# ibejarano/Pynama

Measured on AMD Instinct MI355X. Metric: assembled element-DOFs/sec + CG iterations/sec, 10M-DOF Poisson, 1/2/4/8 MI355X, higher is better.
Workload: dtype f64

## Files before the change

### include/pynama_hip.h

```cpp
#ifndef PYNAMA_HIP_H
#define PYNAMA_HIP_H

#include <stdint.h>

#ifdef __cplusplus
extern "C" {
#endif

typedef struct pyn_ctx pyn_ctx;

enum {
  PYN_OK = 0,
  PYN_EINVAL = -1,
  PYN_EHIP = -2,
  PYN_ENCCL = -3,
  PYN_ENOTCONV = -4,
  PYN_ENOGPU = -5
};

enum { PYN_Q_FULL = 0, PYN_Q_RED = 1, PYN_Q_NODAL = 2 };

enum {
  PYN_FORM_LAPLACE = 0,
  PYN_FORM_MASS_NODAL = 1,
// ... 92 lines not shown
};
#define PYN_FIELD_MAX_PARAMS 4
int pyn_field_info(int field, int* dim, int* bs, int* nparams);
int pyn_field_eval(pyn_ctx* ctx, int field, const double* params, int nparams, int set_id, int vec_id);
int pyn_vec_set_nodes(pyn_ctx* ctx, int vec_id, int set_id, const double* values, int nvalues, const uint8_t* dofs);

int pyn_assemble_kle(pyn_ctx* ctx, double alpha_d, double alpha_w, int K, int Krhs, int Rw, int Rd,
                     int variant);
int pyn_assemble_kle_noslip(pyn_ctx* ctx, double alpha_d, double alpha_w, const int* mat_ids);
int pyn_assemble_scalar(pyn_ctx* ctx, int form, int A, int Arhs, int variant);
int pyn_elem_local(pyn_ctx* ctx, int form, double alpha_d, double alpha_w, const double* corners,
                   double* out0, double* out1, double* out2);

int pyn_assemble_operator(pyn_ctx* ctx, int rule, int nterms, const int32_t* terms, const double* coef, int mat_id);
int pyn_elem_operator_local(pyn_ctx* ctx, int rule, int br, int bc, int nterms, const int32_t* terms,
                            const double* coef, const double* corners, double* out);

int pyn_spmv(pyn_ctx* ctx, int mat_id, int x_vec, int y_vec);
int pyn_product_last(pyn_ctx* ctx, int64_t* info);
int pyn_product_choose(int br, int bc, int npat, int maxw, int64_t nnzb, int64_t n_owned, int rhs_compact, int solver, int image,
                       int sell_image, int block_sell, int no_csrlb, int no_sell, double bcsr_min_avg, int bcsr_lanes, int bcsr_unroll,
                       int* kind, int* W, int* lanes, int* unroll);
int pyn_assemble_last(pyn_ctx* ctx, int64_t* info);
int pyn_assemble_choose(const int64_t* request, const int64_t* facts, const int64_t* knobs, int64_t* out);
int pyn_assemble_choose_layout(char* buf, int len);
enum { PYN_MATFREE_OFF = 0, PYN_MATFREE_LAPLACE = 1, PYN_MATFREE_KLE = 2, PYN_MATFREE_KLE_GENERAL = 3,
       PYN_MATFREE_KLE_NGL3_GENERAL = 4 };
int pyn_matfree_set(pyn_ctx* ctx, int op, double alpha_d, double alpha_w);
int pyn_matfree_apply(pyn_ctx* ctx, int op, int x_vec, int y_vec);
typedef struct pyn_solve_opts {
  int method;
  int pc;
  int norm_type;
  int maxit;
  int restart;
  int fixed_iters;
  int profile;
  int cg_variant;
  int gmres_orthog;
  int matfree;
  double rtol, atol, dtol;
} pyn_solve_opts;
typedef struct pyn_solve_info {
  int iters;
  int reason;
  double rnorm;
// ... 50 lines not shown
```

### pynama_amd/_lib.py

```python
from __future__ import annotations

import ctypes as C
import os
import subprocess
import sys

import numpy as np

_HERE = os.path.dirname(os.path.abspath(__file__))
LIB_PATH = os.environ.get("PYNAMA_LIB_PATH") or os.path.join(_HERE, "libpynama_hip.so")
CSRC = os.path.join(_HERE, "csrc")

Q_FULL, Q_RED, Q_NODAL = 0, 1, 2
FORM_LAPLACE, FORM_MASS_NODAL, FORM_MASS_FULL, FORM_KLE, FORM_OPERATOR = 0, 1, 2, 3, 4
KSP_CG, KSP_GMRES = 0, 1
MATFREE_OFF, MATFREE_LAPLACE, MATFREE_KLE, MATFREE_KLE_GENERAL, MATFREE_KLE_NGL3_GENERAL = 0, 1, 2, 3, 4
PC_NONE, PC_JACOBI, PC_MG = 0, 1, 2
MG_MAX_LEVELS = 16
TS_MAX_STAGES = 8
NORM_PRECONDITIONED, NORM_UNPRECONDITIONED, NORM_NATURAL = 0, 1, 2
T_SYMBOLIC, T_ASSEMBLE, T_SPMV, T_SOLVE = 0, 1, 2, 3
(FIELD_TG2D_VEL, FIELD_TG2D_VORT, FIELD_TG3D_VEL, FIELD_TG3D_VORT, FIELD_TG3D_CONV, FIELD_TG3D_DIFF,
 FIELD_SEN2D_VEL, FIELD_SEN2D_VORT, FIELD_SEN2D_CONV, FIELD_SEN2D_DIFF) = range(10)
FIELD_COUNT, FIELD_MAX_PARAMS = 10, 4


class PynamaHipError(RuntimeError):
    pass


class SolveOpts(C.Structure):
    _fields_ = [("method", C.c_int), ("pc", C.c_int), ("norm_type", C.c_int), ("maxit", C.c_int),
                ("restart", C.c_int), ("fixed_iters", C.c_int), ("profile", C.c_int), ("cg_variant", C.c_int),
# ... 68 lines not shown
    "pyn_vec_axpby": [_P, _I, _D, _I, _D, _I],
    "pyn_vec_pointwise_mult": [_P, _I, _I, _I],
    "pyn_vec_reciprocal": [_P, _I],
    "pyn_vec_vtensv": [_P, _I, _I],
    "pyn_vec_dot": [_P, _I, _I, C.POINTER(_D)],
    "pyn_vec_norm": [_P, _I, _I, C.POINTER(_D)],
    "pyn_vec_maxpy": [_P, _I, _I, _I, _pi32, _pf64],
    "pyn_ts_step_finish": [_P, _I, _I, _pi32, _pf64, _P, _D, _D, C.POINTER(_D)],
    "pyn_nodeset_create": [_P, _L, _P, C.POINTER(_I)],
    "pyn_nodeset_destroy": [_P, _I],
    "pyn_field_info": [_I, C.POINTER(_I), C.POINTER(_I), C.POINTER(_I)],
    "pyn_field_eval": [_P, _I, _pf64, _I, _I, _I],
    "pyn_vec_set_nodes": [_P, _I, _I, _pf64, _I, _P],
    "pyn_assemble_kle": [_P, _D, _D, _I, _I, _I, _I, _I],
    "pyn_assemble_kle_noslip": [_P, _D, _D, C.POINTER(_I)],
    "pyn_assemble_scalar": [_P, _I, _I, _I, _I],
    "pyn_elem_local": [_P, _I, _D, _D, _pf64, _P, _P, _P],
    "pyn_assemble_operator": [_P, _I, _I, _pi32, _pf64, _I],
    "pyn_elem_operator_local": [_P, _I, _I, _I, _I, _pi32, _pf64, _pf64, _pf64],
    "pyn_spmv": [_P, _I, _I, _I],
    "pyn_product_last": [_P, _pi64],
    "pyn_product_choose": [_I] * 4 + [_L, _L] + [_I] * 7 + [_D, _I, _I] + [C.POINTER(_I)] * 4,
    "pyn_assemble_last": [_P, _pi64],
    "pyn_assemble_choose": [_pi64, _pi64, _pi64, _pi64],
    "pyn_assemble_choose_layout": [C.c_char_p, _I],
    "pyn_matfree_apply": [_P, _I, _I, _I],
    "pyn_matfree_set": [_P, _I, _D, _D],
    "pyn_solve": [_P, _I, _I, _I, C.POINTER(SolveOpts), C.POINTER(SolveInfo)],
    "pyn_direct_max_rows": [],
    "pyn_solve_direct": [_P, _I, _I, _I, C.POINTER(SolveInfo)],
    "pyn_direct_band_info": [_P, _I, C.POINTER(_L), C.POINTER(_L), C.POINTER(_L)],
    "pyn_solve_direct_band": [_P, _I, _I, _I, _L, C.POINTER(SolveInfo)],
    "pyn_mg_setup": [_P, _I, C.POINTER(MgOpts)],
    "pyn_mg_info": [_P, _I, C.POINTER(_I), _pi64, _pf64, C.POINTER(_D), C.POINTER(_I)],
    "pyn_mg_apply": [_P, _I, _I, _I],
    "pyn_mg_level_get": [_P, _I, _I, _pf64],
    "pyn_ibm_set": [_P, _I, _I, _L, _pf64, _pf64, _pf64, _pf64],
    "pyn_ibm_interp": [_P, _I, _pf64],
    "pyn_ibm_spread": [_P, _pf64, _I],
    "pyn_ibm_correct": [_P, _I, _pf64, _pf64],
    "pyn_ibm_matrix_get": [_P, _pf64],
    "pyn_ibm_info": [_P, _pi64],
    "pyn_ibm_clear": [_P],
    "pyn_probe_create": [_P, _L, _pf64, C.POINTER(_I)],
    "pyn_probe_info": [_P, _I, _pi64],
    "pyn_probe_get": [_P, _I, _pi32, _pf64],
# ... 2 lines not shown
    "pyn_timers_get": [_P, _pf64, _I],
}

_lib = None


def build_library(force=False):
    if force:
        subprocess.check_call(["make", "-C", CSRC, "clean"])
    subprocess.check_call(["make", "-C", CSRC, "-j4"])
    return LIB_PATH


def load_library():
    global _lib
    if _lib is not None:
        return _lib
    if not os.path.exists(LIB_PATH):
        raise PynamaHipError(
            f"{LIB_PATH} not found: build it with `python -c 'import __graft_entry__ as g; g.build()'` "
            "(or `make -C pynama_amd/csrc`). pynama_amd has no CPU fallback.")
    lib = C.CDLL(LIB_PATH)
    for name, args in SIGNATURES.items():
        fn = getattr(lib, name)
        fn.argtypes = args
        fn.restype = C.c_int
    for name in ("pyn_last_error", "pyn_source_hash"):
        getattr(lib, name).argtypes = []
        getattr(lib, name).restype = C.c_char_p
    _lib = lib
    return lib


def _check(rc):
    if rc != 0:
        raise PynamaHipError(f"[{rc}] {_lib.pyn_last_error().decode(errors='replace')}")


def source_hash() -> str:
    return load_library().pyn_source_hash().decode()


def alloc_live():
    n, b = _L(0), _L(0)
    _check(load_library().pyn_alloc_live(C.byref(n), C.byref(b)))
    return n.value, b.value
# ... 425 lines not shown
        _check(self.lib.pyn_elem_local(self.h, form, 0.0, 0.0, c, o0.ctypes.data_as(_P), None, None))
        return o0

    def assemble_operator(self, rule, terms, coef, mid):
        t = _i32(terms).reshape(-1, 3)
        _check(self.lib.pyn_assemble_operator(self.h, rule, t.shape[0], t, _f64(coef), mid))

    def elem_operator_local(self, rule, br, bc, terms, coef, corners):
        t = _i32(terms).reshape(-1, 3)
        out = np.empty((br * self.nn, bc * self.nn))
        _check(self.lib.pyn_elem_operator_local(self.h, rule, br, bc, t.shape[0], t, _f64(coef), _f64(corners).ravel(), out))
        return out

    def spmv(self, mid, x, y):
        _check(self.lib.pyn_spmv(self.h, mid, x, y))

    def product_last(self):
        info = np.zeros(8, np.int64)
        _check(self.lib.pyn_product_last(self.h, info))
        keys = ("family", "param", "unroll", "dot", "grid", "npat", "maxw", "launches")
        return {k: int(v) for k, v in zip(keys, info)}

    def assemble_last(self):
        info = np.zeros(8, np.int64)
        _check(self.lib.pyn_assemble_last(self.h, info))
        return {k: int(v) for k, v in zip(_ASM_LAST_KEYS, info)}

    def mesh_ho_lattice(self):
        g, a, b, c = _I(0), _I(0), _I(0), _I(0)
        _check(self.lib.pyn_mesh_ho_lattice(self.h, C.byref(g), C.byref(a), C.byref(b), C.byref(c)))
        return g.value, a.value, b.value, c.value

    def matfree_apply(self, x, y, op=1):
        _check(self.lib.pyn_matfree_apply(self.h, op, x, y))

    def matfree_set(self, op=1, alpha_d=0.0, alpha_w=0.0):
        _check(self.lib.pyn_matfree_set(self.h, op, alpha_d, alpha_w))

    def matfree_kle_set(self, alpha_d, alpha_w):
        self.matfree_set(MATFREE_KLE, alpha_d, alpha_w)

    def solve(self, mid, b, x, method=KSP_CG, pc=PC_JACOBI, rtol=1e-5, atol=1e-50, dtol=1e5, maxit=10000,
              restart=30, norm_type=NORM_PRECONDITIONED, fixed_iters=0, profile=0, cg_variant=0, gmres_orthog=0,
              matfree=0) -> SolveInfo:
        o = SolveOpts(method, pc, norm_type, maxit, restart, fixed_iters, profile, cg_variant, gmres_orthog, matfree,
                      rtol, atol, dtol)
        info = SolveInfo()
        _check(self.lib.pyn_solve(self.h, mid, b, x, C.byref(o), C.byref(info)))
        return info
# ... 132 lines not shown
```

### pynama_amd/csrc/pyn_assemble.hip

```cpp
#include <cstring>

#include "pyn_internal.h"

namespace {

struct AsmArgs {
  const int32_t* conn;
  const double* xyz;
  int64_t n_elem, n_owned;
  int dim, nn, nc;
  int ngp[3];
  const double* w[3];
  const double* H[3];
  const double* Hrs[3];
  const double* HrsCoo[3];
  const int32_t* rowptr;
  const int32_t* colidx;
  const uint8_t* bcmask;
  int form;
  double alpha_d, alpha_w;
  double *K, *Krhs, *Rw, *Rd;
  double *Kfs, *Krhsfs, *Rwfs, *Rdfs;
  const int32_t *rcrow, *rcrow_fs;
  const int32_t* esel;
// ... 950 lines not shown
}

int zero_blocks(pyn_ctx* c, double* val, int64_t blocks, int br, int bc) {
  if (val) PYN_HIP(hipMemsetAsync(val, 0, (size_t)blocks * br * bc * sizeof(double), c->stream));
  return PYN_OK;
}

void launch_bc_identity(pyn_ctx* c, int ndof, double* K, double* Krhs, double* Kfs, double* Krhsfs, const int32_t* rcrow,
                        const int32_t* rcrow_fs) {
  const int64_t n = c->n_owned * ndof;
  const int grid = (int)std::min<int64_t>((n + 255) / 256, 4096);
  bc_identity_kernel<<<grid, 256, 0, c->stream>>>(c->d_rowptr, c->d_colidx, c->d_bcmask, c->n_owned, ndof, K, Krhs, Kfs, Krhsfs, rcrow, rcrow_fs);
}

int asm_finish(pyn_ctx* c, const AsmPlan& P, const AsmRequest& rq) {
  PYN_HIP(hipEventRecord(c->ev1, c->stream));
  PYN_HIP(hipStreamSynchronize(c->stream));
  float ms = 0;
  PYN_HIP(hipEventElapsedTime(&ms, c->ev0, c->ev1));
  c->timers[PYN_T_ASSEMBLE] = ms;
  const int64_t r[7] = {P.kind, P.shape, P.k_closed, P.rw_closed, P.kind == AK_GENERIC ? rq.generic : 0, rq.krhs_completed, rq.dinv_written};
  std::copy(r, r + 7, c->asm_last);
  c->asm_last[7] += 1;
  return PYN_OK;
}

bool rowrun_asked(const AsmRequest& rq) {
  if (rq.variant == 0 || rq.Rd) return false;
  return rq.form == PYN_FORM_KLE ? rq.K || (rq.Rw && !rq.Krhs) : rq.form == PYN_FORM_LAPLACE && rq.K && !rq.Rw;
}
bool rowrun_static(const AsmRequest& rq, const AsmFacts& f, const AsmKnobs& k) {
  if (!f.ho3_valid || f.ho3_tabs_nn != f.nn || f.ngp0 < 1) return false;
  if (rq.form == PYN_FORM_OPERATOR)
    return rq.op_rule == PYN_Q_NODAL && f.ho3_tabs_ok2 && rq.op_nterms <= PYN_HO3_MAX_TERMS && !k.no_ho3_operator;
  return rowrun_asked(rq) && f.ho3_tabs_ok0 && !(f.ngl == 2 && f.dim == 3) && (rq.form != PYN_FORM_KLE || f.ho3_tabs_ok1);
}
bool lattice_static(const AsmRequest& rq, const AsmFacts& f) {
  return rq.variant != 0 && rq.form == PYN_FORM_LAPLACE && rq.K && !rq.Rw && !rq.Rd && f.lat_valid && !f.plan0_user && f.ngp0 == 8;
}
bool kle_lattice_static(const AsmRequest& rq, const AsmFacts& f, const AsmKnobs& k) {
  return rq.variant != 0 && rq.form == PYN_FORM_KLE && (rq.K || (rq.Rw && !rq.Krhs)) && !rq.Rd && !f.plan1_user && f.lat_valid &&
         f.ngp0 == 8 && f.ngp1 == 1 && !k.no_kle_lattice;
}
bool patch_static(const AsmRequest& rq, const AsmFacts& f, const AsmKnobs& k) {
  if (rq.variant == 0 || !rq.K || rq.Rd || f.dim != 3) return false;
  if (rq.form == PYN_FORM_KLE) return f.nn == 8 && f.ngp0 == 8 && f.ngp1 == 1;
// ... 272 lines not shown
  rq.variant = variant;
  rq.rhs_clean = Arhs != Aid && rhs_is_clean(c, k, Arhs);
  PYN_TRY(mat_ptr(c, Aid, 1, 1, "A", &rq.K));
  PYN_TRY(mat_ptr(c, Arhs, 1, 1, "Arhs", &rq.Krhs, &rq.rcrow));
  if (rq.rcrow) rq.rhs_clean = false;
  rq.krhs_blocks = rhs_blocks(c, Arhs);
  if (Aid >= 0 && form == PYN_FORM_LAPLACE && !k.no_dinv) {
    DMat& m = c->mats[Aid];
    if (!m.dinv) PYN_HIP(m.dinv.alloc((size_t)c->n_owned));
    rq.dinv = m.dinv;
  }
  PYN_TRY(asm_run(c, rq, k));
  if (rq.dinv_written) c->mats[Aid].dinv_valid = true;
  if (rq.Krhs && rq.K) c->mats[Arhs].rhs_clean = c->bc_stamp;
  return PYN_OK;
}

extern "C" int pyn_assemble_last(pyn_ctx* c, int64_t* info) {
  PYN_CHECK(c && info, "NULL argument");
  std::copy(c->asm_last, c->asm_last + 8, info);
  return PYN_OK;
}

#define PYN_ASM_REQUEST "form,variant,K,Krhs,Rw,Rd,krhs_compact,op_rule,op_nterms"
extern "C" int pyn_assemble_choose_layout(char* buf, int len) {
#define PYN_X(f) #f ","
#define PYN_F(f, e) #f ","
#define PYN_I(f, e, d) #f ","
  const char* layout = "request:" PYN_ASM_REQUEST ";facts:" PYN_ASM_FACTS(PYN_X) ";knobs:" PYN_ASM_KNOBS(PYN_F, PYN_I);
#undef PYN_X
#undef PYN_F
#undef PYN_I
  PYN_CHECK(buf && len > (int)strlen(layout), "pyn_assemble_choose_layout: the buffer needs %zu bytes", strlen(layout) + 1);
  strcpy(buf, layout);
  return PYN_OK;
}

extern "C" int pyn_assemble_choose(const int64_t* request, const int64_t* facts, const int64_t* knobs, int64_t* out) {
  PYN_CHECK(request && facts && knobs && out, "pyn_assemble_choose: NULL argument");
  static double target;
  static const int32_t crow = 0;
  AsmRequest rq;
  rq.form = (int)request[0];
  rq.variant = (int)request[1];
  rq.K = request[2] ? &target : nullptr;
  rq.Krhs = request[3] ? &target : nullptr;
// ... 121 lines not shown
```

### pynama_amd/csrc/pyn_assemble_lattice.hip

```cpp
#include "pyn_internal.h"
#include "pyn_q1_hex.h"
#include "pyn_lattice.h"

namespace {


__device__ __forceinline__ double lat_affine_inv(const double* __restrict__ S, const double (&E)[3][3], double (&Ji)[3][3]) {
  double J[3][3];
#pragma unroll
  for (int d = 0; d < 3; ++d)
#pragma unroll
    for (int x = 0; x < 3; ++x) J[d][x] = fma(S[d * 3 + 2], E[2][x], fma(S[d * 3 + 1], E[1][x], S[d * 3] * E[0][x]));
  const double c00 = J[1][1] * J[2][2] - J[1][2] * J[2][1];
  const double c01 = J[1][2] * J[2][0] - J[1][0] * J[2][2];
  const double c02 = J[1][0] * J[2][1] - J[1][1] * J[2][0];
  const double det = J[0][0] * c00 + J[0][1] * c01 + J[0][2] * c02;
  const double r = 1.0 / det;
  Ji[0][0] = c00 * r;
  Ji[0][1] = (J[0][2] * J[2][1] - J[0][1] * J[2][2]) * r;
  Ji[0][2] = (J[0][1] * J[1][2] - J[0][2] * J[1][1]) * r;
  Ji[1][0] = c01 * r;
  Ji[1][1] = (J[0][0] * J[2][2] - J[0][2] * J[2][0]) * r;
  Ji[1][2] = (J[0][2] * J[1][0] - J[0][0] * J[1][2]) * r;
  Ji[2][0] = c02 * r;
// ... 413 lines not shown
          pA[m] = fr ? idv : (fc ? 0.0 : v);
          if (pR) pR[m] = fr ? idv : (fc ? -v : 0.0);
        }
        lat_rows_step(p, st, cc);
      }
    }
    if (tid < 4 * cc) {
      const LatRowsEnd r = lat_rows_end(tid, nx, cc, len);
      const double2 k = skx[3 * r.x + r.dx + 1], c = abl[r.t];
      const unsigned fr = fself[r.x], fc = fll[r.t * W + r.x + r.dx + 1];
      const double v = fma(k.x, c.x, k.y * c.y);
      const double idv = (r.t == tself && r.dx == 0) ? 1.0 : 0.0;
      outA[r.e] = fr ? idv : (fc ? 0.0 : v);
      if (outR && (zeros || fr || fc)) outR[r.e] = fr ? idv : (fc ? -v : 0.0);
    }
    if (T.dinv) {
      const double2 c = abl[tself];
      double* __restrict__ dv = T.dinv + ((int64_t)zo * ny + y) * nx;
      for (int x = tid; x < nx; x += NT) {
        const double2 k = skx[x * 3 + 1];
        dv[x] = fself[x] ? 1.0 : 1.0 / fma(k.x, c.x, k.y * c.y);
      }
    }
  }
}

struct HaarQ {
  double xx, yy, zz, xy, xz, yz;
};
__device__ __forceinline__ HaarQ haar_q(const double (&Ji)[3][3], const double det) {
  const double d8 = 0.125 * det;
  HaarQ q;
  q.xx = d8 * (Ji[0][0] * Ji[0][0] + Ji[1][0] * Ji[1][0] + Ji[2][0] * Ji[2][0]);
  q.yy = d8 * (Ji[0][1] * Ji[0][1] + Ji[1][1] * Ji[1][1] + Ji[2][1] * Ji[2][1]);
  q.zz = d8 * (Ji[0][2] * Ji[0][2] + Ji[1][2] * Ji[1][2] + Ji[2][2] * Ji[2][2]);
  q.xy = d8 * (Ji[0][0] * Ji[0][1] + Ji[1][0] * Ji[1][1] + Ji[2][0] * Ji[2][1]);
  q.xz = d8 * (Ji[0][0] * Ji[0][2] + Ji[1][0] * Ji[1][2] + Ji[2][0] * Ji[2][2]);
  q.yz = d8 * (Ji[0][1] * Ji[0][2] + Ji[1][1] * Ji[1][2] + Ji[2][1] * Ji[2][2]);
  return q;
}
constexpr int HAAR_NODE[2][2][2] = {{{0, 4}, {1, 7}}, {{3, 5}, {2, 6}}};

template <int S>
__device__ __forceinline__ void haar_fwd(const double* xe, double (&g)[2][2][2]) {
  double h[2][2][2];
#pragma unroll
// ... 1291 lines not shown
    return PYN_OK;
  }
  DevBuf<double> tab;
  DevTmp flag;
  PYN_HIP(tab.alloc((size_t)lat_rows_tab_base(B.NX, B.NY, B.npl) + lat_rows_tab_doubles(B.NX, B.NY, B.npl)));
  PYN_HIP(flag.alloc(sizeof(int)));
  const int one = 1;
  PYN_HIP(hipMemcpyAsync(flag.get(), &one, sizeof(int), hipMemcpyHostToDevice, c->stream));
  LatArgs Tc;
  lat_fill(c, k, Tc);
  lattice_axes_extract_kernel<<<(ns + 255) / 256, 256, 0, c->stream>>>(Tc, tab);
  lattice_axes_check_kernel<<<(int)((n_node + 255) / 256), 256, 0, c->stream>>>(Tc, tab, n_node, flag.as<int>());
  lattice_rows_tables_kernel<<<(B.NX + B.NY + B.npl + 255) / 256, 256, 0, c->stream>>>(Tc, tab);
  PYN_HIP(hipGetLastError());
  int h = 0;
  PYN_HIP(hipMemcpyAsync(&h, flag.get(), sizeof(int), hipMemcpyDeviceToHost, c->stream));
  PYN_HIP(hipStreamSynchronize(c->stream));
  if (h) L.d_axes = std::move(tab);
  L.rect = h ? 1 : 0;
  return PYN_OK;
}

template <int NL, int NT>
static int launch_lattice_rows(pyn_ctx* c, LatArgs& T) {
  const size_t lds = lat_rows_lds(T.nx, NL);
  const int64_t n_groups = (int64_t)((T.ny + NL - 1) / NL) * T.n_own;
  PYN_CHECK(n_groups > 0 && n_groups < (int64_t)INT32_MAX, "lattice rows kernel: %lld workgroups", (long long)n_groups);
  const double* km = c->lat.d_axes.get() + lat_rows_tab_base(T.nx, T.ny, T.npl);
  assemble_q1_lattice_rows_kernel<NL, NT><<<(int)n_groups, NT, lds, c->stream>>>(T, km);
  PYN_HIP(hipGetLastError());
  return PYN_OK;
}

static int lat_fill_args(pyn_ctx* c, LatArgs& T, int* mesh_aff) {
  const AsmKnobs k = lat_fill_knobs();
  PYN_TRY(pyn_lattice_checks(c, k));
  lat_fill(c, k, T);
  *mesh_aff = c->mesh_affine == 1;
  return PYN_OK;
}

static void kle_fill(const pyn_ctx* c, KleLatArgs& T, double alpha_d, double alpha_w) {
  T.alpha_d = alpha_d;
  T.alpha_w = alpha_w;
  T.wr = c->quad[1].w;
  T.hrsr = c->quad[1].Hrs;
  T.Hr = c->quad[1].H;
  T.hcoor = c->quad[1].HrsCoo;
}

template <int TX, int TY, int TZ, bool GEN>
static int launch_kle_lattice(pyn_ctx* c, KleLatArgs& T, double* K, double* Krhs, double* Rw) {
  using LT = LatTile<TX, TY, TZ>;
// ... 56 lines not shown
      T.axX = c->lat.d_axes;
      T.axY = T.axX + lat_axis_slots(T.nx);
      T.axZ = T.axY + lat_axis_slots(T.ny);
    }
  }
  PYN_CHECK(!k.lattice_axes_require || T.axX,
            "PYNAMA_LATTICE_AXES_REQUIRE: the axis-table variant of the lattice tile kernel does not apply (%s)",
            !tiles_closed ? "not the parallelepiped tile kernel" : k.no_lattice_axes || k.lattice_ablate == 32 ? "switched off"
                                                                                                              : "mesh not rectilinear");
  int rows_nl = k.lattice_rows_lines == 2 ? 2 : 1;
  while (rows_nl > 1 && lat_rows_lds(T.nx, rows_nl) > 64 * 1024) rows_nl /= 2;
  const char* no_rows = !tiles_closed                                                                ? "not the parallelepiped tile kernel"
                        : k.no_lattice_rows                                                          ? "switched off"
                        : k.lattice_tile >= 0                                                        ? "PYNAMA_LATTICE_TILE asks for a tile shape"
                        : k.lattice_ablate != 0                                                      ? "PYNAMA_LATTICE_ABLATE is set"
                        : k.no_lattice_axes || k.lattice_axes_require || k.no_lattice_tilebc         ? "a switch of the tile kernel's variants is set"
                        : rq.rcrow                                                                   ? "compact Arhs"
                        : c->lat.rect != 1                                                           ? "mesh not rectilinear"
                        : lat_rows_lds(T.nx, rows_nl) > 64 * 1024                                            ? "x-lines too long for the LDS staging"
                                                                                                     : nullptr;
  PYN_CHECK(!k.lattice_rows_require || !no_rows, "PYNAMA_LATTICE_ROWS_REQUIRE: the rows kernel of rectilinear lattices does not apply (%s)",
            no_rows);
  if (!no_rows) {
    if (rows_nl == 2) return launch_lattice_rows<2, 256>(c, T);
    switch (k.lattice_rows_threads) {
      case 128: return launch_lattice_rows<1, 128>(c, T);
      case 512: return launch_lattice_rows<1, 512>(c, T);
      default: return launch_lattice_rows<1, 256>(c, T);
    }
  }
  if (k.lattice_ablate == 64) T.bcmask = nullptr;
  if (P.kind == AK_MARCH) return pyn_assemble_lattice_march(c, k, &T, P.shape);
  const bool affine = P.k_closed, tilebc = !k.no_lattice_tilebc;
  switch (P.shape) {
    case 1: return launch_lattice<7, 7, 7>(c, T, affine, tilebc);
    case 2: return launch_lattice<6, 6, 6>(c, T, affine, tilebc);
    case 3: return launch_lattice<8, 6, 6>(c, T, affine, tilebc);
    case 4: return launch_lattice<7, 6, 6>(c, T, affine, tilebc);
    case 5: return launch_lattice<6, 6, 4>(c, T, affine, tilebc);
    case 6: return launch_lattice<6, 5, 5>(c, T, affine, tilebc);
    case 7: return launch_lattice<7, 4, 4>(c, T, affine, tilebc);
    case 8: return launch_lattice<14, 3, 3>(c, T, affine, tilebc);
    case 9: return launch_lattice<7, 5, 5>(c, T, affine, tilebc);
    default: return launch_lattice<7, 5, 4>(c, T, affine, tilebc);
  }
}


static int mf_select_layers(LatArgs& T, int ntz, int zsel) {
  const int lo = T.p_own0 > 0 ? 1 : 0, hi = T.p_own0 + T.n_own < T.npl ? 1 : 0;
  T.bz0 = 0;
// ... 211 lines not shown
```

### pynama_amd/csrc/pyn_ctx.hip

```cpp
#include <fcntl.h>
#include <sched.h>
#include <sys/mman.h>
#include <sys/stat.h>
#include <unistd.h>

#include <atomic>
#include <chrono>
#include <cstdarg>
#include <cstring>

#include "pyn_internal.h"

struct pyn_shm_hdr {
  std::atomic<int> count;
  std::atomic<int> sense;
  int nranks;
  int64_t cap;
  std::atomic<int> hcount;
  std::atomic<int> hsense;
};
struct pyn_shm_comm {
  unsigned char* base = nullptr;
  size_t size = 0;
  int rank = 0, nranks = 1, local_sense = 0, halo_sense = 0;
// ... 465 lines not shown

__global__ void box_xyz_kernel(BoxArgs B, double* __restrict__ xyz) {
  const int64_t n = (int64_t)blockIdx.x * blockDim.x + threadIdx.x;
  if (n >= B.n_node) return;
  const int64_t k = n / B.PS, in = n - k * B.PS;
  const int64_t g = B.planes[k];
  if (B.dim == 3) {
    const int iy = (int)(in / B.N[0]), ix = (int)(in - (int64_t)iy * B.N[0]);
    xyz[n * 3] = B.axes[ix];
    xyz[n * 3 + 1] = B.axes[B.N[0] + iy];
    xyz[n * 3 + 2] = B.axes[B.N[0] + B.N[1] + g];
  } else {
    xyz[n * 2] = B.axes[in];
    xyz[n * 2 + 1] = B.axes[B.N[0] + g];
  }
}

static int mesh_installed(pyn_ctx* c, const ConnAt& at) {
  c->mesh_affine = -1;
  c->lat.rect = -1;
  c->lat.d_axes.reset();
  c->lat.d_tilebc.reset();
  c->lat.tilebc_stamp = -1;
  for (int k = 0; k < PYN_MATFREE_SLOTS; ++k) {
    c->mf_mask[k].reset();
    c->mf_set[k] = false;
  }
  c->ibm.reset();
  for (auto& s : c->nodesets) s = DNodeSet();
  for (auto& p : c->probes) p = DProbe();
  c->d_probe_loc.reset();
  c->d_probe_tab.reset();
  c->probe_tab_ngl = c->probe_tab_dim = 0;
  c->d_rowptr.reset();
  c->d_colidx.reset();
  c->nnzb = 0;
  {
    DevBuf<unsigned long long> d_bad;
    unsigned long long bad = ~0ull;
    const int64_t n = c->n_elem * c->nn;
    PYN_HIP(d_bad.alloc(1));
    PYN_HIP(hipMemcpyAsync(d_bad, &bad, sizeof(bad), hipMemcpyHostToDevice, c->stream));
    conn_range_kernel<<<(unsigned)std::min<int64_t>((n + 255) / 256, 4096), 256, 0, c->stream>>>(c->d_conn, n, (int32_t)c->n_node, d_bad);
    PYN_HIP(hipGetLastError());
    PYN_HIP(hipMemcpyAsync(&bad, d_bad, sizeof(bad), hipMemcpyDeviceToHost, c->stream));
    PYN_HIP(hipStreamSynchronize(c->stream));
// ... 619 lines not shown
```

### pynama_amd/csrc/pyn_internal.h

```cpp
#pragma once
#include <hip/hip_runtime.h>
#include <rccl/rccl.h>

#include <algorithm>
#include <atomic>
#include <cstdint>
#include <cstdio>
#include <functional>
#include <map>
#include <memory>
#include <string>
#include <type_traits>
#include <utility>
#include <vector>

#include "../../include/pynama_hip.h"

void pyn_set_error(const char* fmt, ...);

#define PYN_HIP(call)                                                                         \
  do {                                                                                        \
    hipError_t e_ = (call);                                                                   \
    if (e_ != hipSuccess) {                                                                   \
      pyn_set_error("%s:%d %s -> %s", __FILE__, __LINE__, #call, hipGetErrorString(e_));      \
// ... 175 lines not shown
  DevBuf<int32_t> d_P;
  std::vector<int32_t> P;
  int64_t plane() const { return (int64_t)NX * NY; }
  int ny() const { return dim == 3 ? NY : npl; }
  int nz() const { return dim == 3 ? npl : 1; }
  bool slab_order() const {
    bool ok = true;
    for (int j = 0; j < npl && ok; ++j) ok = P[j] == (j < p_own0 ? n_own + j : (j >= p_own0 + n_own ? j : j - p_own0)) * plane();
    return ok;
  }
  bool natural() const { return p_own0 == 0 && n_own == npl && slab_order(); }
};

struct Lattice {
  bool valid = false;
  bool std_shape = false;
  int std_ok = -1;
  DevBuf<int32_t> d_zord;
  int rect = -1;
  DevBuf<double> d_axes;
  DevBuf<uint32_t> d_tilebc;
  int64_t tilebc_stamp = -1;
  int tilebc_shape = -1;
};

struct Ho3View {
  bool valid = false;
  int affine = -1;
  int diag = 0;
  DevBuf<double> d_geom;
  DevBuf<uint8_t> d_nbits;
  int64_t nbits_stamp = -1;
  DevBuf<uint8_t> d_runflag;
  int64_t runflag_stamp = -1;
  int runflag_R = 0;
};

struct Ho3MfBasis {
  double Bf[3][3], Gf[3][3];
  double Br[2][3], Gr[2][3];
  double C[3][3];
  int diag = 0;
};

constexpr int PYN_MATFREE_SLOTS = PYN_MATFREE_KLE_NGL3_GENERAL + 1;
constexpr int PYN_HO_MAX_NGL_2D = 12, PYN_HO_MAX_NGL_3D = 8;
// ... 124 lines not shown
  std::vector<SellShape> sell_shapes;
  DevBuf<int32_t> sell_pid;
  DevBuf<int32_t> sell_tab;
  int sell_npat = 0;
  bool sell_dict_built = false;
  int64_t prod_last[8] = {0};

  std::vector<DMat> mats;
  std::vector<DVec> vecs;
  std::vector<DNodeSet> nodesets;
  std::vector<DProbe> probes;
  DevBuf<int32_t> d_probe_loc;
  DevBuf<double> d_probe_tab;
  int probe_tab_ngl = 0, probe_tab_dim = 0;

  DevBuf<double> d_part;
  DevBuf<double> d_scal;
  DevBuf<int> d_flag;
  PinBuf<double> h_scal;
  PinBuf<int> h_flag;
  DevBuf<double> d_work;
  std::vector<hipEvent_t> prof_ev;
  int64_t asm_last[8] = {0};
  std::map<const void*, size_t> kern_lds;
  std::map<std::pair<const void*, size_t>, int> kern_occ;
  DevBuf<int32_t> d_esel;
  int64_t n_esel = 0, esel_stamp = -1;
  DevBuf<double> d_kle_lel;
  DevBuf<double> d_eloc;
  std::unique_ptr<IbmState, IbmStateDelete> ibm;
};

inline int64_t n_local(const pyn_ctx* c) { return c->n_owned + c->n_ghost; }
inline void pyn_product_record(pyn_ctx* c, ProductKind family, int p1, int p2, bool dot, int grid, int maxw) {
  int64_t* r = c->prod_last;
  r[0] = family;
  r[1] = p1;
  r[2] = p2;
  r[3] = dot ? 1 : 0;
  r[4] = grid;
  r[5] = c->sell_npat;
  r[6] = maxw;
  r[7] += 1;
}
inline int pyn_lattice_kind(const pyn_ctx* c) {
  if (c->ho3.valid && (c->box.ngl == 3 || c->box.dim == 2)) return c->box.ngl == 3 ? 2 : 3;
// ... 73 lines not shown
int pyn_mg_ensure(pyn_ctx* c, DMat& A);
int pyn_mg_vcycle(pyn_ctx* c, DMat& A, const double* r, double* z, const LinOp& prod0);

enum AssemblyKind { AK_NONE = 0, AK_GENERIC = 1, AK_P1 = 2, AK_PATCH = 3, AK_LATTICE = 4, AK_MARCH = 5, AK_KLE_LATTICE = 6, AK_ROWRUN = 7 };
constexpr int PYN_HO3_MAX_TERMS = 32;

#define PYN_LAT_FILL_KNOBS(F, I)                                                                                                 \
  F(no_affine, "PYNAMA_NO_AFFINE") F(no_lean, "PYNAMA_NO_LEAN") F(no_std_lattice, "PYNAMA_NO_STD_LATTICE")                       \
  I(lattice_ablate, "PYNAMA_LATTICE_ABLATE", 0)
#define PYN_ASM_KNOBS(F, I)                                                                                                      \
  PYN_LAT_FILL_KNOBS(F, I) F(no_lean_plan, "PYNAMA_NO_LEAN_PLAN") F(no_p1, "PYNAMA_NO_P1")                                       \
  F(no_p1_tiled, "PYNAMA_NO_P1_TILED") F(no_ho, "PYNAMA_NO_HO") F(no_ho_mfma, "PYNAMA_NO_HO_MFMA")                               \
  F(no_dinv, "PYNAMA_NO_ASM_DINV") F(rhs_full_write, "PYNAMA_RHS_FULL_WRITE")                                                    \
  F(no_kle_lattice, "PYNAMA_NO_KLE_LATTICE") F(no_kle_general, "PYNAMA_NO_KLE_GENERAL") F(no_march, "PYNAMA_NO_MARCH")           \
  F(no_ho3_lattice, "PYNAMA_NO_HO3_LATTICE") F(no_ho3_operator, "PYNAMA_NO_HO3_OPERATOR") F(ho3_require, "PYNAMA_HO3_REQUIRE")   \
  F(ho3_no_diag, "PYNAMA_HO3_NO_DIAG") F(ho3_no_pstd, "PYNAMA_HO3_NO_PSTD") F(march_stamps, "PYNAMA_MARCH_STAMPS")               \
  I(lattice_tile, "PYNAMA_LATTICE_TILE", -1) I(march_tile, "PYNAMA_MARCH_TILE", -1)                                             \
  I(kle_lattice_tile, "PYNAMA_KLE_LATTICE_TILE", -1) I(march_zlen, "PYNAMA_MARCH_ZLEN", -1) I(ho3_run, "PYNAMA_HO3_RUN", 0)     \
  I(ho3_wgs_per_cu, "PYNAMA_HO3_WGS_PER_CU", -1) I(ho3_grid, "PYNAMA_HO3_GRID", -1) I(kle_ablate, "PYNAMA_KLE_ABLATE", 0)       \
  I(tiled_ablate, "PYNAMA_TILED_ABLATE", 0) I(ho3_ablate, "PYNAMA_HO3_ABLATE", 0)
#define PYN_ASM_LAUNCH_KNOBS(F, I) F(no_lattice_axes, "PYNAMA_NO_LATTICE_AXES") F(lattice_axes_require, "PYNAMA_LATTICE_AXES_REQUIRE") \
  F(no_lattice_tilebc, "PYNAMA_NO_LATTICE_TILEBC") F(no_lattice_rows, "PYNAMA_NO_LATTICE_ROWS")                                      \
  F(lattice_rows_require, "PYNAMA_LATTICE_ROWS_REQUIRE") I(lattice_rows_lines, "PYNAMA_LATTICE_ROWS_LINES", 0)               \
  I(lattice_rows_threads, "PYNAMA_LATTICE_ROWS_THREADS", 0)
struct AsmKnobs {
#define PYN_F(f, e) bool f = false;
#define PYN_I(f, e, d) int f = d;
  PYN_ASM_KNOBS(PYN_F, PYN_I)
  PYN_ASM_LAUNCH_KNOBS(PYN_F, PYN_I)
#undef PYN_F
#undef PYN_I
};
AsmKnobs asm_knobs();
AsmKnobs lat_fill_knobs();

#define PYN_ASM_FACTS(X)                                                                                                         \
  X(dim) X(nn) X(nc) X(ngl) X(ngp0) X(ngp1) X(ngp2) X(const_grad) X(q1_gauss_standard) X(q1_red_standard) X(aff_standard)        \
  X(aff_rw_standard) X(mesh_affine) X(lat_valid) X(lat_std_ok) X(ho3_valid) X(ho3_affine) X(ho3_tabs_nn) X(ho3_tabs_ok0)         \
  X(ho3_tabs_ok1) X(ho3_tabs_ok2) X(plan0_present) X(plan0_user) X(plan0_unfit) X(plan1_present) X(plan1_user) X(plan1_unfit)
struct AsmFacts {
#define PYN_X(f) int f = 0;
  PYN_ASM_FACTS(PYN_X)
#undef PYN_X
  bool geom_done = false, plan_declined = false;
};

struct AsmRequest {
  int form = 0, variant = 1;
  double alpha_d = 0.0, alpha_w = 0.0;
  double *K = nullptr, *Krhs = nullptr, *Rw = nullptr, *Rd = nullptr;
  const int32_t* rcrow = nullptr;
  int64_t krhs_blocks = 0;
  bool rhs_clean = false;
  double* dinv = nullptr;
  int op_rule = 0, op_br = 0, op_bc = 0, op_nterms = 0;
  const int32_t* op_terms = nullptr;
  const double* op_coef = nullptr;
  bool dinv_written = false;
  bool krhs_completed = false;
  int generic = 0;
};

struct AsmPlan {
  AssemblyKind kind = AK_GENERIC;
  int shape = 0;
  bool k_closed = false, rw_closed = false;
  bool kle_general = false;
  int generic = 0;
  bool krhs_pending = false;
  bool dinv = false;
  bool rowrun_candidate = false, want_plan = false;
};
AsmPlan asm_choose(const AsmRequest& rq, const AsmFacts& f, const AsmKnobs& k);
int asm_facts(pyn_ctx* c, const AsmRequest& rq, const AsmKnobs& k, AsmFacts* f);
int pyn_assemble_ho3_lattice(pyn_ctx* c, const AsmRequest& rq, const AsmKnobs& k, const AsmPlan& P);
int pyn_assemble_lattice(pyn_ctx* c, AsmRequest& rq, const AsmKnobs& k, const AsmPlan& P);
int pyn_assemble_lattice_march(pyn_ctx* c, const AsmKnobs& k, void* lat_args, int shape);
int pyn_assemble_kle_lattice(pyn_ctx* c, const AsmRequest& rq, const AsmKnobs& k, const AsmPlan& P);
int pyn_assemble_patch(pyn_ctx* c, const AsmRequest& rq, const AsmKnobs& k, const AsmPlan& P);
int pyn_patch_plan_default(pyn_ctx* c, int kind);
int pyn_lattice_checks(pyn_ctx* c, const AsmKnobs& k);
int pyn_ho3_prepare(pyn_ctx* c);
int pyn_ho3_run_length(int dim, int ngl, bool op, int knob);
// ... 5 lines not shown
```

### pynama_amd/csrc/pyn_lattice_rows.h

```cpp
#pragma once
#include <cstdint>

#include "pyn_lattice_axes.h"

PYN_AX_HD inline int lat_rows_plane(int nx, int ny, int p_own0, int n_own, int j) {
  const int pp = nx * ny, lo = p_own0, hi = p_own0 + n_own;
  if (j < lo) return (n_own + j) * pp;
  if (j >= hi) return (n_own + lo + (j - hi)) * pp;
  return (j - lo) * pp;
}

PYN_AX_HD inline int lat_rows_zcode(int npl, int p_own0, int n_own, int pl) {
  const int lo = p_own0, hi = p_own0 + n_own;
  const bool has_dn = pl > 0, has_up = pl < npl - 1;
  const bool dn_ghost = has_dn && pl - 1 < lo, up_ghost = has_up && pl + 1 >= hi;
  int code = 0, n = 0;
  if (has_dn && !dn_ghost) code |= 0 << (2 + 2 * n++);
  code |= 1 << (2 + 2 * n++);
  if (has_up && !up_ghost) code |= 2 << (2 + 2 * n++);
  if (dn_ghost) code |= 0 << (2 + 2 * n++);
  if (up_ghost) code |= 2 << (2 + 2 * n++);
  return code | n;
}

// ... 41 lines not shown
PYN_AX_HD inline void lat_rows_step(LatRowsPos& p, const LatRowsStride& s, int cc) {
  p.kx += s.ks;
  const int c1 = p.kx >= 3;
  p.kx -= c1 ? 3 : 0;
  p.t += s.rs + c1;
  const int c2 = p.t >= cc;
  p.t -= c2 ? cc : 0;
  p.x += s.qs + c2;
}

struct LatRowsEnd {
  int e, x, t, dx;
};
PYN_AX_HD inline LatRowsEnd lat_rows_end(int j, int nx, int cc, int len) {
  const int last = j >= 2 * cc, jj = j - (last ? 2 * cc : 0);
  LatRowsEnd r;
  r.e = last ? len - 2 * cc + jj : jj;
  r.x = last ? nx - 1 : 0;
  r.t = jj >> 1;
  r.dx = (jj & 1) - last;
  return r;
}

PYN_AX_HD inline int lat_rows_tab_base(int nx, int ny, int npl) {
  return (lat_axis_slots(nx) + lat_axis_slots(ny) + lat_axis_slots(npl) + 1) & ~1;
}
PYN_AX_HD inline int lat_rows_tab_doubles(int nx, int ny, int npl) { return 6 * (nx + ny + npl); }
PYN_AX_HD inline void lat_rows_km(const double* c, int i, int n, double* km) {
  const bool lo = i > 0, hi = i < n - 1;
  double hm = lo ? c[i] - c[i - 1] : 0.0, hp = hi ? c[i + 1] - c[i] : 0.0;
  hm = hm < 0.0 ? -hm : hm;
  hp = hp < 0.0 ? -hp : hp;
  const double rm = lo ? 1.0 / hm : 0.0, rp = hi ? 1.0 / hp : 0.0;
  km[0] = -rm;
  km[1] = hm / 6.0;
  km[2] = rm + rp;
  km[3] = (hm + hp) / 3.0;
  km[4] = -rp;
  km[5] = hp / 6.0;
}
```

Baseline: 196.5 billion.

## Add persistent line-walking lattice rows assembly kernel with cached BC class map

Adds a persistent-style rows assembly kernel where each workgroup walks several x-lines. It loads the x-axis stencil table into LDS once per workgroup and stages per-line coefficients and boundary flags. A cached per-line boundary-class map, rebuilt only when BCs change, lets lines with no interior Dirichlet nodes skip the per-node mask reads and handle only edge entries from the bit word. This is meant to cut repeated mask loads and per-workgroup setup, but it adds a map pass and more complex scheduling, and the grid is capped only when the max-grid knob is set.

Measured after the change: 205.1 billion (median of 6 runs). +4.4%, better.

```diff
diff --git a/include/pynama_hip.h b/include/pynama_hip.h
--- a/include/pynama_hip.h
+++ b/include/pynama_hip.h
@@ -138,6 +138,7 @@
                        int sell_image, int block_sell, int no_csrlb, int no_sell, double bcsr_min_avg, int bcsr_lanes, int bcsr_unroll,
                        int* kind, int* W, int* lanes, int* unroll);
 int pyn_assemble_last(pyn_ctx* ctx, int64_t* info);
+int pyn_assemble_last_rows(pyn_ctx* ctx, int64_t* info);
 int pyn_assemble_choose(const int64_t* request, const int64_t* facts, const int64_t* knobs, int64_t* out);
 int pyn_assemble_choose_layout(char* buf, int len);
 enum { PYN_MATFREE_OFF = 0, PYN_MATFREE_LAPLACE = 1, PYN_MATFREE_KLE = 2, PYN_MATFREE_KLE_GENERAL = 3,
diff --git a/pynama_amd/_lib.py b/pynama_amd/_lib.py
--- a/pynama_amd/_lib.py
+++ b/pynama_amd/_lib.py
@@ -8,7 +8,9 @@
 import numpy as np
 
 _HERE = os.path.dirname(os.path.abspath(__file__))
-LIB_PATH = os.environ.get("PYNAMA_LIB_PATH") or os.path.join(_HERE, "libpynama_hip.so")
+_DEFAULT_LIB_PATH = os.path.join(_HERE, "libpynama_hip.so")
+LIB_PATH = os.environ.get("PYNAMA_LIB_PATH") or _DEFAULT_LIB_PATH
+_NEWER_SYMBOLS = ("pyn_assemble_last_rows",)
 CSRC = os.path.join(_HERE, "csrc")
 
 Q_FULL, Q_RED, Q_NODAL = 0, 1, 2
@@ -123,6 +125,7 @@
     "pyn_product_last": [_P, _pi64],
     "pyn_product_choose": [_I] * 4 + [_L, _L] + [_I] * 7 + [_D, _I, _I] + [C.POINTER(_I)] * 4,
     "pyn_assemble_last": [_P, _pi64],
+    "pyn_assemble_last_rows": [_P, _pi64],
     "pyn_assemble_choose": [_pi64, _pi64, _pi64, _pi64],
     "pyn_assemble_choose_layout": [C.c_char_p, _I],
     "pyn_matfree_apply": [_P, _I, _I, _I],
@@ -171,6 +174,8 @@
             "(or `make -C pynama_amd/csrc`). pynama_amd has no CPU fallback.")
     lib = C.CDLL(LIB_PATH)
     for name, args in SIGNATURES.items():
+        if name in _NEWER_SYMBOLS and LIB_PATH != _DEFAULT_LIB_PATH and not hasattr(lib, name):
+            continue
         fn = getattr(lib, name)
         fn.argtypes = args
         fn.restype = C.c_int
@@ -642,9 +647,13 @@
         return {k: int(v) for k, v in zip(keys, info)}
 
     def assemble_last(self):
-        info = np.zeros(8, np.int64)
+        info, rows = np.zeros(8, np.int64), np.zeros(2, np.int64)
         _check(self.lib.pyn_assemble_last(self.h, info))
-        return {k: int(v) for k, v in zip(_ASM_LAST_KEYS, info)}
+        if hasattr(self.lib, "pyn_assemble_last_rows"):
+            _check(self.lib.pyn_assemble_last_rows(self.h, rows))
+        else:
+            rows[:] = -1
+        return dict({k: int(v) for k, v in zip(_ASM_LAST_KEYS, info)}, rows_form=int(rows[0]), rows_grid=int(rows[1]))
 
     def mesh_ho_lattice(self):
         g, a, b, c = _I(0), _I(0), _I(0), _I(0)
diff --git a/pynama_amd/csrc/pyn_assemble.hip b/pynama_amd/csrc/pyn_assemble.hip
--- a/pynama_amd/csrc/pyn_assemble.hip
+++ b/pynama_amd/csrc/pyn_assemble.hip
@@ -996,6 +996,8 @@
   const int64_t r[7] = {P.kind, P.shape, P.k_closed, P.rw_closed, P.kind == AK_GENERIC ? rq.generic : 0, rq.krhs_completed, rq.dinv_written};
   std::copy(r, r + 7, c->asm_last);
   c->asm_last[7] += 1;
+  c->asm_last_rows[0] = rq.rows_form;
+  c->asm_last_rows[1] = rq.rows_grid;
   return PYN_OK;
 }
 
@@ -1314,6 +1316,12 @@
   return PYN_OK;
 }
 
+extern "C" int pyn_assemble_last_rows(pyn_ctx* c, int64_t* info) {
+  PYN_CHECK(c && info, "NULL argument");
+  std::copy(c->asm_last_rows, c->asm_last_rows + 2, info);
+  return PYN_OK;
+}
+
 #define PYN_ASM_REQUEST "form,variant,K,Krhs,Rw,Rd,krhs_compact,op_rule,op_nterms"
 extern "C" int pyn_assemble_choose_layout(char* buf, int len) {
 #define PYN_X(f) #f ","
diff --git a/pynama_amd/csrc/pyn_assemble_lattice.hip b/pynama_amd/csrc/pyn_assemble_lattice.hip
--- a/pynama_amd/csrc/pyn_assemble_lattice.hip
+++ b/pynama_amd/csrc/pyn_assemble_lattice.hip
@@ -459,6 +459,187 @@
         dv[x] = fself[x] ? 1.0 : 1.0 / fma(k.x, c.x, k.y * c.y);
       }
     }
+  }
+}
+
+__global__ void __launch_bounds__(64) lattice_rows_map_kernel(LatArgs T, uint32_t* __restrict__ map) {
+  __shared__ uint32_t bits;
+  const int line = blockIdx.x, y = line % T.ny, pl = T.p_own0 + line / T.ny;
+  if (threadIdx.x == 0) bits = 0;
+  __syncthreads();
+  const uint32_t mine = lat_rows_line_bits(T.nx, T.ny, y, lat_zcode(T, pl), (int)threadIdx.x, 64, [&](int dy, int dz, int x) {
+    return T.bcmask[(int64_t)lat_plane(T, pl + dz) + (int64_t)(y + dy) * T.nx + x] != 0;
+  });
+  if (mine) atomicOr(&bits, mine);
+  __syncthreads();
+  if (threadIdx.x == 0) map[line] = lat_rows_word(bits);
+}
+
+static size_t lat_rows_walk_lds(int nx) {
+  return (size_t)nx * 48 + 144 + (((size_t)9 * (nx + 2) + 15) & ~(size_t)15);
+}
+
+struct LatRowsLine {
+  int y, zo, zcode;
+  uint32_t word;
+  int64_t base;
+};
+
+template <int NT, bool STD>
+__global__ void __launch_bounds__(NT, 2048 / NT) __attribute__((amdgpu_num_sgpr(80)))
+assemble_q1_lattice_rows_walk_kernel(LatArgs T, const double* __restrict__ km, const uint32_t* __restrict__ lmap, int n_lines) {
+  extern __shared__ __align__(16) double lds[];
+  const int tid = threadIdx.x, nx = T.nx, ny = T.ny, W = nx + 2;
+  double2* skx = reinterpret_cast<double2*>(lds);
+  double2* abl = skx + 3 * nx;
+  unsigned char* fll = reinterpret_cast<unsigned char*>(abl + 9);
+  const double2* __restrict__ kmx = reinterpret_cast<const double2*>(km);
+  const double2* __restrict__ kmy = kmx + 3 * nx;
+  const double2* __restrict__ kmz = kmy + 3 * ny;
+  const uint32_t no_map = T.bcmask ? 2u : 0u;
+
+  auto fetch = [&](int line) {
+    LatRowsLine L;
+    L.y = line % ny;
+    L.zo = line / ny;
+    L.zcode = lat_zcode<STD>(T, T.p_own0 + L.zo);
+    L.word = lmap ? lmap[line] : no_map;
+    L.base = STD ? lat_rowptr_std(T, 0, L.y, L.zo) : T.rowptr[(int64_t)T.P[T.p_own0 + L.zo] + (int64_t)L.y * nx];
+    return L;
+  };
+  auto stage = [&](const LatRowsLine& L) {
+    const int y = L.y, pl = T.p_own0 + L.zo, cy = 3 - (y == 0) - (y == ny - 1), cc = cy * (L.zcode & 3);
+    if (lat_rows_class(L.word) == 2) {
+      int rowoff;
+      {
+        int dy, dz;
+        lat_rows_group(min(min(tid & 63, 8), cc - 1), cy, y != 0, L.zcode, dy, dz);
+        rowoff = lat_plane<STD>(T, pl + dz) + (y + dy) * nx;
+      }
+      for (int i0 = 0; i0 < W; i0 += NT) {
+        const int i = i0 + tid, xi = min(max(i - 1, 0), nx - 1);
+        unsigned char f[9];
+#pragma unroll
+        for (int s = 0; s < 9; ++s) f[s] = T.bcmask[(int64_t)__builtin_amdgcn_readlane(rowoff, s) + xi];
+        if (i < W) {
+          const bool inx = i >= 1 && i <= nx;
+#pragma unroll
+          for (int s = 0; s < 9; ++s) fll[s * W + i] = (inx && f[s] != 0) ? 1 : 0;
+        }
+      }
+    }
+    const double2 y0 = kmy[y * 3], y1 = kmy[y * 3 + 1], y2 = kmy[y * 3 + 2];
+    const double2 z0 = kmz[pl * 3], z1 = kmz[pl * 3 + 1], z2 = kmz[pl * 3 + 2];
+    if (tid < cc) {
+      int dy, dz;
+      lat_rows_group(tid, cy, y != 0, L.zcode, dy, dz);
+      const double2 fy = dy < 0 ? y0 : dy == 0 ? y1 : y2, fz = dz < 0 ? z0 : dz == 0 ? z1 : z2;
+      abl[tid] = make_double2(fy.y * fz.y, fma(fy.x, fz.y, fy.y * fz.x));
+    }
+  };
+
+  auto store = [&](const LatRowsLine& L) {
+    const int y = L.y, zo = L.zo, zcode = L.zcode, cy = 3 - (y == 0) - (y == ny - 1), cz = zcode & 3, cc = cy * cz;
+    const int tself = ((zcode >> 2) & 3) == 1 ? (y != 0) : cy + (y != 0);
+    double* __restrict__ outA = T.A + L.base;
+    double* __restrict__ outR = T.Arhs ? T.Arhs + L.base : nullptr;
+    const bool zeros = outR && !T.rhs_clean;
+    const int len = lat_rows_line_len(nx, cy, cz), nint = lat_rows_interior_len(nx, cc);
+    const uint32_t magic = lat_rows_magic(cc);
+    double* __restrict__ dv = T.dinv ? T.dinv + ((int64_t)zo * ny + y) * nx : nullptr;
+    if (lat_rows_class(L.word) == 2) {
+      const unsigned char* fself = fll + tself * W + 1;
+      if (tid < nint) {
+        const LatRowsStride st = lat_rows_stride(NT, cc);
+        LatRowsPos p = lat_rows_interior(tid, cc, magic);
+        double* __restrict__ pA = outA + 2 * cc;
+        double* __restrict__ pR = outR ? outR + 2 * cc : nullptr;
+        for (int m = tid; m < nint; m += NT) {
+          const double2 k = skx[__mul24(p.x, 3) + p.kx], c = abl[p.t];
+          const unsigned fr = fself[p.x], fc = fll[__mul24(p.t, W) + p.x + p.kx];
+          const double v = fma(k.x, c.x, k.y * c.y);
+          if (!__any(fr | fc)) {
+            pA[m] = v;
+            if (zeros) pR[m] = 0.0;
+          } else {
+            const double idv = (p.t == tself && p.kx == 1) ? 1.0 : 0.0;
+            pA[m] = fr ? idv : (fc ? 0.0 : v);
+            if (pR) pR[m] = fr ? idv : (fc ? -v : 0.0);
+          }
+          lat_rows_step(p, st, cc);
+        }
+      }
+      if (tid < 4 * cc) {
+        const LatRowsEnd r = lat_rows_end(tid, nx, cc, len);
+        const double2 k = skx[3 * r.x + r.dx + 1], c = abl[r.t];
+        const unsigned fr = fself[r.x], fc = fll[r.t * W + r.x + r.dx + 1];
+        const double v = fma(k.x, c.x, k.y * c.y);
+        const double idv = (r.t == tself && r.dx == 0) ? 1.0 : 0.0;
+        outA[r.e] = fr ? idv : (fc ? 0.0 : v);
+        if (outR && (zeros || fr || fc)) outR[r.e] = fr ? idv : (fc ? -v : 0.0);
+      }
+      if (dv) {
+        const double2 c = abl[tself];
+        for (int x = tid; x < nx; x += NT) {
+          const double2 k = skx[x * 3 + 1];
+          dv[x] = fself[x] ? 1.0 : 1.0 / fma(k.x, c.x, k.y * c.y);
+        }
+      }
+      return;
+    }
+    const int nfree = nint - 6 * cc;
+    if (tid < nfree) {
+      const LatRowsStride st = lat_rows_stride(NT, cc);
+      LatRowsPos p = lat_rows_interior(3 * cc + tid, cc, magic);
+      double* __restrict__ pA = outA + 5 * cc;
+      double* __restrict__ pR = outR ? outR + 5 * cc : nullptr;
+      for (int m = tid; m < nfree; m += NT) {
+        const double2 k = skx[__mul24(p.x, 3) + p.kx], c = abl[p.t];
+        pA[m] = fma(k.x, c.x, k.y * c.y);
+        if (zeros) pR[m] = 0.0;
+        lat_rows_step(p, st, cc);
+      }
+    }
+    auto edge = [&](int e, int x, int t, int dx) {
+      const double2 k = skx[3 * x + dx + 1], c = abl[t];
+      const unsigned fr = lat_rows_word_flag(L.word, tself, x, nx), fc = lat_rows_word_flag(L.word, t, x + dx, nx);
+      const double v = fma(k.x, c.x, k.y * c.y);
+      const double idv = (t == tself && dx == 0) ? 1.0 : 0.0;
+      outA[e] = fr ? idv : (fc ? 0.0 : v);
+      if (outR && (zeros || fr || fc)) outR[e] = fr ? idv : (fc ? -v : 0.0);
+    };
+    const int nedge = min(nint, 6 * cc);
+    if (tid < nedge) {
+      const int m = tid < 3 * cc ? tid : nint - 6 * cc + tid;
+      const LatRowsPos p = lat_rows_interior(m, cc, magic);
+      edge(2 * cc + m, p.x, p.t, p.kx - 1);
+    }
+    if (tid < 4 * cc) {
+      const LatRowsEnd r = lat_rows_end(tid, nx, cc, len);
+      edge(r.e, r.x, r.t, r.dx);
+    }
+    if (dv) {
+      const double2 c = abl[tself];
+      for (int x = tid; x < nx; x += NT) {
+        const double2 k = skx[x * 3 + 1];
+        dv[x] = lat_rows_word_flag(L.word, tself, x, nx) ? 1.0 : 1.0 / fma(k.x, c.x, k.y * c.y);
+      }
+    }
+  };
+
+  int line = lat_rows_sched(blockIdx.x, gridDim.x, n_lines, 0);
+  if (line < 0) return;
+  LatRowsLine L = fetch(line);
+  for (int q = tid; q < 3 * nx; q += NT) skx[q] = kmx[q];
+  stage(L);
+  for (int trip = 1;; ++trip) {
+    __syncthreads();
+    store(L);
+    line = lat_rows_sched(blockIdx.x, gridDim.x, n_lines, trip);
+    if (line < 0) break;
+    L = fetch(line);
+    __syncthreads();
+    stage(L);
   }
 }
 
@@ -1796,13 +1977,52 @@
 }
 
 template <int NL, int NT>
-static int launch_lattice_rows(pyn_ctx* c, LatArgs& T) {
+static int launch_lattice_rows(pyn_ctx* c, LatArgs& T, AsmRequest& rq) {
   const size_t lds = lat_rows_lds(T.nx, NL);
   const int64_t n_groups = (int64_t)((T.ny + NL - 1) / NL) * T.n_own;
   PYN_CHECK(n_groups > 0 && n_groups < (int64_t)INT32_MAX, "lattice rows kernel: %lld workgroups", (long long)n_groups);
   const double* km = c->lat.d_axes.get() + lat_rows_tab_base(T.nx, T.ny, T.npl);
   assemble_q1_lattice_rows_kernel<NL, NT><<<(int)n_groups, NT, lds, c->stream>>>(T, km);
   PYN_HIP(hipGetLastError());
+  rq.rows_form = 1;
+  rq.rows_grid = (int)n_groups;
+  return PYN_OK;
+}
+
+static int lattice_rows_map_ensure(pyn_ctx* c, const LatArgs& T, int n_lines) {
+  Lattice& L = c->lat;
+  if (L.d_rowsmap && L.rowsmap_stamp == c->bc_stamp) return PYN_OK;
+  DevBuf<uint32_t> map;
+  PYN_HIP(map.alloc((size_t)n_lines));
+  lattice_rows_map_kernel<<<n_lines, 64, 0, c->stream>>>(T, map);
+  PYN_HIP(hipGetLastError());
+  L.d_rowsmap = std::move(map);
+  L.rowsmap_stamp = c->bc_stamp;
+  return PYN_OK;
+}
+
+template <bool STD>
+static int launch_lattice_rows_walk(pyn_ctx* c, const AsmKnobs& k, LatArgs& T, AsmRequest& rq) {
+  const size_t lds = lat_rows_walk_lds(T.nx);
+  const int64_t n_lines = (int64_t)T.ny * T.n_own;
+  PYN_CHECK(n_lines > 0 && n_lines < (int64_t)INT32_MAX, "lattice rows kernel: %lld x-lines", (long long)n_lines);
+  const uint32_t* lmap = nullptr;
+  if (T.bcmask && !k.lattice_rows_no_classes) {
+    PYN_TRY(lattice_rows_map_ensure(c, T, (int)n_lines));
+    lmap = c->lat.d_rowsmap;
+  }
+  int64_t grid = n_lines;
+  if (k.lattice_rows_max_grid > 0) grid = std::min<int64_t>(grid, k.lattice_rows_max_grid);
+  if (k.lattice_rows_max_grid < 0) {
+    int per_cu = 0;
+    PYN_TRY(pyn_kernel_occupancy(c, reinterpret_cast<const void*>(assemble_q1_lattice_rows_walk_kernel<256, STD>), 256, lds, &per_cu));
+    grid = std::min<int64_t>(grid, (int64_t)std::max(1, per_cu) * 256);
+  }
+  const double* km = c->lat.d_axes.get() + lat_rows_tab_base(T.nx, T.ny, T.npl);
+  assemble_q1_lattice_rows_walk_kernel<256, STD><<<(int)grid, 256, lds, c->stream>>>(T, km, lmap, (int)n_lines);
+  PYN_HIP(hipGetLastError());
+  rq.rows_form = 2;
+  rq.rows_grid = (int)grid;
   return PYN_OK;
 }
 
@@ -1905,11 +2125,13 @@
   PYN_CHECK(!k.lattice_rows_require || !no_rows, "PYNAMA_LATTICE_ROWS_REQUIRE: the rows kernel of rectilinear lattices does not apply (%s)",
             no_rows);
   if (!no_rows) {
-    if (rows_nl == 2) return launch_lattice_rows<2, 256>(c, T);
+    if (!k.lattice_rows_oneshot && rows_nl == 1 && k.lattice_rows_threads == 0 && lat_rows_walk_lds(T.nx) <= 64 * 1024)
+      return T.std_lat ? launch_lattice_rows_walk<true>(c, k, T, rq) : launch_lattice_rows_walk<false>(c, k, T, rq);
+    if (rows_nl == 2) return launch_lattice_rows<2, 256>(c, T, rq);
     switch (k.lattice_rows_threads) {
-      case 128: return launch_lattice_rows<1, 128>(c, T);
-      case 512: return launch_lattice_rows<1, 512>(c, T);
-      default: return launch_lattice_rows<1, 256>(c, T);
+      case 128: return launch_lattice_rows<1, 128>(c, T, rq);
+      case 512: return launch_lattice_rows<1, 512>(c, T, rq);
+      default: return launch_lattice_rows<1, 256>(c, T, rq);
     }
   }
   if (k.lattice_ablate == 64) T.bcmask = nullptr;
diff --git a/pynama_amd/csrc/pyn_ctx.hip b/pynama_amd/csrc/pyn_ctx.hip
--- a/pynama_amd/csrc/pyn_ctx.hip
+++ b/pynama_amd/csrc/pyn_ctx.hip
@@ -511,6 +511,8 @@
   c->lat.d_axes.reset();
   c->lat.d_tilebc.reset();
   c->lat.tilebc_stamp = -1;
+  c->lat.d_rowsmap.reset();
+  c->lat.rowsmap_stamp = -1;
   for (int k = 0; k < PYN_MATFREE_SLOTS; ++k) {
     c->mf_mask[k].reset();
     c->mf_set[k] = false;
diff --git a/pynama_amd/csrc/pyn_internal.h b/pynama_amd/csrc/pyn_internal.h
--- a/pynama_amd/csrc/pyn_internal.h
+++ b/pynama_amd/csrc/pyn_internal.h
@@ -221,6 +221,8 @@
   DevBuf<uint32_t> d_tilebc;
   int64_t tilebc_stamp = -1;
   int tilebc_shape = -1;
+  DevBuf<uint32_t> d_rowsmap;
+  int64_t rowsmap_stamp = -1;
 };
 
 struct Ho3View {
@@ -391,6 +393,7 @@
   DevBuf<double> d_work;
   std::vector<hipEvent_t> prof_ev;
   int64_t asm_last[8] = {0};
+  int64_t asm_last_rows[2] = {0};
   std::map<const void*, size_t> kern_lds;
   std::map<std::pair<const void*, size_t>, int> kern_occ;
   DevBuf<int32_t> d_esel;
@@ -510,7 +513,8 @@
 #define PYN_ASM_LAUNCH_KNOBS(F, I) F(no_lattice_axes, "PYNAMA_NO_LATTICE_AXES") F(lattice_axes_require, "PYNAMA_LATTICE_AXES_REQUIRE") \
   F(no_lattice_tilebc, "PYNAMA_NO_LATTICE_TILEBC") F(no_lattice_rows, "PYNAMA_NO_LATTICE_ROWS")                                      \
   F(lattice_rows_require, "PYNAMA_LATTICE_ROWS_REQUIRE") I(lattice_rows_lines, "PYNAMA_LATTICE_ROWS_LINES", 0)               \
-  I(lattice_rows_threads, "PYNAMA_LATTICE_ROWS_THREADS", 0)
+  I(lattice_rows_threads, "PYNAMA_LATTICE_ROWS_THREADS", 0) F(lattice_rows_oneshot, "PYNAMA_LATTICE_ROWS_ONESHOT")                      \
+  I(lattice_rows_max_grid, "PYNAMA_LATTICE_ROWS_MAX_GRID", 0) F(lattice_rows_no_classes, "PYNAMA_LATTICE_ROWS_NO_CLASSES")
 struct AsmKnobs {
 #define PYN_F(f, e) bool f = false;
 #define PYN_I(f, e, d) int f = d;
@@ -547,6 +551,7 @@
   bool dinv_written = false;
   bool krhs_completed = false;
   int generic = 0;
+  int rows_form = 0, rows_grid = 0;
 };
 
 struct AsmPlan {
diff --git a/pynama_amd/csrc/pyn_lattice_rows.h b/pynama_amd/csrc/pyn_lattice_rows.h
--- a/pynama_amd/csrc/pyn_lattice_rows.h
+++ b/pynama_amd/csrc/pyn_lattice_rows.h
@@ -87,6 +87,34 @@
   return r;
 }
 
+PYN_AX_HD inline int lat_rows_sched(int wg, int grid, int n, int trip) {
+  const int ng = grid < 8 ? grid : 8, j = wg % ng, w = wg / ng;
+  const int g = (grid - j + ng - 1) / ng;
+  const int q = n / ng, r = n % ng, cnt = q + (j < r);
+  const int64_t i = w + (int64_t)trip * g;
+  return i < cnt ? j * q + (j < r ? j : r) + (int)i : -1;
+}
+
+PYN_AX_HD inline uint32_t lat_rows_node_bits(int x, int nx, int t, bool imposed) {
+  return !imposed ? 0u : x == 0 ? 1u << (2 + t) : x == nx - 1 ? 1u << (11 + t) : 1u << 31;
+}
+template <class F>
+PYN_AX_HD inline uint32_t lat_rows_line_bits(int nx, int ny, int y, int zcode, int x0, int xstep, F imposed) {
+  const int cy = 3 - (y == 0) - (y == ny - 1), cc = cy * (zcode & 3);
+  uint32_t bits = 0;
+  for (int t = 0; t < cc; ++t) {
+    int dy, dz;
+    lat_rows_group(t, cy, y != 0, zcode, dy, dz);
+    for (int x = x0; x < nx; x += xstep) bits |= lat_rows_node_bits(x, nx, t, imposed(dy, dz, x));
+  }
+  return bits;
+}
+PYN_AX_HD inline uint32_t lat_rows_word(uint32_t bits) { return (bits & 0x7ffffffcu) | ((bits >> 31) ? 2u : bits ? 1u : 0u); }
+PYN_AX_HD inline int lat_rows_class(uint32_t word) { return (int)(word & 3u); }
+PYN_AX_HD inline unsigned lat_rows_word_flag(uint32_t word, int t, int xx, int nx) {
+  return xx == 0 ? (word >> (2 + t)) & 1u : xx == nx - 1 ? (word >> (11 + t)) & 1u : 0u;
+}
+
 PYN_AX_HD inline int lat_rows_tab_base(int nx, int ny, int npl) {
   return (lat_axis_slots(nx) + lat_axis_slots(ny) + lat_axis_slots(npl) + 1) & ~1;
 }
```
